# ZenGo-X/zk-paillier

Measured on AMD Instinct MI355X. Metric: RangeProofNi proofs/sec + verifies/sec, n=2048, batch=4096 per GPU (value = verifies/sec; proofs/sec in prove.value), higher is better.
Workload: dtype u32 (29-bit limbs, u64 accumulate)

## Files before the change

### zk-paillier_amd/csrc/kernels_basen.hpp

```cpp
#pragma once
#include "kernels_modexp.hpp"

#define ZKP_UNROLL_STR(x) #x
#define ZKP_UNROLL_(n) _Pragma(ZKP_UNROLL_STR(unroll n))
#define ZKP_UNROLL(n) ZKP_UNROLL_(n)
#ifndef ZKP_BN_ROW_UNROLL
#if ZKP_W == 9
#define ZKP_BN_ROW_UNROLL 8
#else
#define ZKP_BN_ROW_UNROLL 1
#endif
#endif
#ifndef ZKP_BN_ASM
#define ZKP_BN_ASM (ZKP_W == 36)
#endif
namespace zkp {
template <int G> constexpr bool BN_ASM_G = ZKP_BN_ASM && W == 36 && (G == 2 || G == 4);

template <int G> struct BnConst {
  static constexpr int L = Geo<G>::L;
  static constexpr int OFF_MT = 0, OFF_C3 = L, OFF_RRA = 2 * L, OFF_RRB = 3 * L, OFF_N = 4 * L, OFF_R2N = 5 * L, OFF_ONE = 6 * L, OFF_R1A = 7 * L, OFF_R1B = 8 * L, OFF_NI = 9 * L, OFF_OK = 9 * L + 1;
  static constexpr int WORDS = 9 * L + 4;
  static constexpr int STRIDE = WORDS + 2 * L;
};
// ... 533 lines not shown
  store_limbs_global<G>(tab + L, Y, g.gl);
  bn_stage<G>(g, g.A(), X);
  bn_stage<G>(g, g.B(), Y);
  const int msb = 31 - __clz(CAP);
#pragma unroll 1
  for (int b = msb - 1; b >= 0; b--) {
    bn_square<G>(g, X);
    if ((CAP >> b) & 1) {
      uint32_t A2[W], B2[W];
      bn_product<G>(g, A2, B2, tab, tab + L);
      bn_stage<G>(g, g.A(), A2);
      bn_stage<G>(g, g.B(), B2);
#pragma unroll
      for (int k = 0; k < W; k++) X[k] = A2[k];
    }
  }
  lds_load_block(Y, g.B() + g.gl * BLK);
  store_limbs_global<G>(out + BC::OFF_RRA, X, g.gl);
  store_limbs_global<G>(out + BC::OFF_RRB, Y, g.gl);
  store_limbs_global<G>(out + BC::OFF_R1A, OA, g.gl);
  store_limbs_global<G>(out + BC::OFF_R1B, OB, g.gl);
  if (g.gl == 0) {
    out[BC::OFF_OK] = ok ? 1u : 0u;
    if (!ok) atomicAnd(all_ok, 0u);
  }
  if (tag && up_tag && gid == 0 && g.gl == 0) {
    tag[1] = up_tag[5];
    __threadfence();
    tag[0] = (ok && up_tag[0] == SETUP_TAG_MAGIC) ? SETUP_TAG_MAGIC : 0u;
  }
}

template <int GS>
__global__ void __launch_bounds__(256, ZKP_WPE) k_expected(EncArgs a, uint32_t* __restrict__ expected, const uint32_t* __restrict__ bn_ok) {
  using CL = ConstLayout<GS>;
  using LL = LdsLayout<GS>;
  if (!*bn_ok) return;
  extern __shared__ __align__(16) uint32_t lds_raw[];
  Grp<GS> g;
  grp_init<GS>(g, lds_raw);
  const int kw = a.n_bits / 32;
  const uint64_t count = a.count_ptr ? (uint64_t)*a.count_ptr : a.count;
  const uint64_t stride = (uint64_t)gridDim.x * LL::GROUPS_PER_BLOCK;
  const uint64_t rounds = (count + stride - 1) / stride;
  const uint32_t* cst = a.consts;
  load_modulus_consts<GS>(g, cst);
  for (uint64_t rd = 0; rd < rounds; rd++) {
    const uint64_t idx = rd * stride + (uint64_t)blockIdx.x * LL::GROUPS_PER_BLOCK + (threadIdx.x / GS);
    const bool live = idx < count;
    const uint64_t item = live ? idx : count - 1;
    uint64_t b;
    bool mask_row;
    const uint32_t* pexp;
    if (a.mode == 2) { b = item; mask_row = a.cipher_x != nullptr; pexp = a.c1 + item * 2 * kw; }
    else {
      b = a.item_proof[item];
      const uint32_t rw = a.item_row[item];
      const uint64_t row = b * a.ef + (rw >> 1);
      mask_row = a.resp_kind[row] != 0;
      const bool use_c1 = mask_row ? (a.resp_j[row] == 1) : !(rw & 1);
      pexp = (use_c1 ? a.c1 : a.c2) + row * 2 * kw;
    }
    if (a.const_stride) {
      const uint64_t i0 = (a.mode == 0 && a.half && item >= a.half) ? item - a.half : item;
      cst = a.consts + (a.mode == 1 ? b : i0 / a.items_per_key) * a.const_stride;
      load_modulus_consts<GS>(g, cst);
    }
    const bool valid = cst[CL::OFF_ST] == 0;
    uint32_t A[W], R[W], Y[W];
    load_value<GS>(g, A, pexp, valid ? 2 * kw : 0);
    stage_const<GS>(g, cst + CL::OFF_R2);
    mm<GS>(g, R, A);
    {
      uint32_t t[W];
      load_value<GS>(g, t, a.cipher_x + b * 2 * kw, (mask_row && valid) ? 2 * kw : 0);
      if (!mask_row && valid && g.gl == 0) t[0] = 1;
      stageB<GS>(g, t);
    }
    mm<GS>(g, Y, R);
    stage_const<GS>(g, cst + CL::OFF_R2);
    mm<GS>(g, R, Y);
    stage_one<GS>(g);
    mm<GS>(g, Y, R);
    canonical_words<GS>(g, Y, cst + CL::OFF_N);
    if (live && mask_row) for (int w = g.gl; w < 2 * kw; w += GS) expected[item * 2 * kw + w] = g.words()[w];
  }
}

struct BnItem {
  const uint32_t* pm; const uint32_t* pr; const uint32_t* pexp; uint32_t* pout;
  uint64_t b; int mw, rw; bool mask_row;
};
__device__ __forceinline__ BnItem bn_item(const EncArgs& a, uint64_t item, const uint32_t* expected) {
  BnItem it{};
  const int kw = a.n_bits / 32;
  it.mw = kw; it.rw = kw;
  if (a.mode == 0) {
    const bool second = a.half && item >= a.half;
    const uint64_t i = second ? item - a.half : item;
    it.mw = a.m_words < 0 ? 0 : (a.m_words ? a.m_words : kw);
    it.rw = a.r_words ? a.r_words : kw;
    it.pm = (second ? a.m2 : a.m) + i * it.mw;
    it.pr = (second ? a.r2 : a.r) + i * it.rw;
    it.pout = (second ? a.out2 : a.out) + i * 2 * kw;
  } else if (a.mode == 2) {
    it.b = item;
    it.pm = a.m + item * kw;
    it.pr = a.r + item * kw;
    it.mask_row = a.cipher_x != nullptr;
    it.pexp = it.mask_row ? expected + item * 2 * kw : a.c1 + item * 2 * kw;
  } else {
    it.b = a.item_proof[item];
    const uint32_t rw = a.item_row[item];
    const uint64_t row = it.b * a.ef + (rw >> 1);
    it.mask_row = a.resp_kind[row] != 0;
    const bool second = (rw & 1) != 0;
    it.pm = (second ? a.resp_w2 : a.resp_w1) + row * kw;
    it.pr = (second ? a.resp_r2 : a.resp_r1) + row * kw;
// ... 568 lines not shown
```

### zk-paillier_amd/csrc/kernels_proofs.hpp

```cpp
#pragma once
#include "kernels_modexp.hpp"
#include "kernels_gcd.hpp"
#include "sha256_dev.hpp"

namespace zkp {

__device__ __forceinline__ int cmp_words(const uint32_t* a, const uint32_t* b, int n) {
  for (int i = n - 1; i >= 0; i--) {
    const uint32_t x = a[i], y = b[i];
    if (x != y) return x > y ? 1 : -1;
  }
  return 0;
}

__device__ __forceinline__ int challenge_bit(const uint8_t* e, uint32_t i) { return (e[i >> 3] >> (7 - (i & 7))) & 1; }

struct RangeHashArgs {
  const uint32_t* n; uint64_t n_stride;
  const uint32_t* c1; const uint32_t* c2; const uint32_t* range;
  uint32_t kw, ef; uint64_t batch;
  uint8_t* e;
  uint8_t* e_len;
  uint32_t* third;
  uint32_t* two_thirds;
// ... 243 lines not shown
  const uint8_t* db = reinterpret_cast<const uint8_t*>(s.row);
  int lead = 0;
  while (lead < 31 && db[lead] == 0) lead++;
  uint8_t* e = a.e + b * 32;
  for (int i = 0; i < 32; i++) e[i] = (i + lead < 32) ? db[i + lead] : 0;
  const int elen = 32 - lead;
  a.e_len[b] = (uint8_t)elen;
  a.verdict[b] = ((uint32_t)elen * 8 >= a.ef) ? a.ok_value : (uint8_t)ZKP_VERDICT_MALFORMED;
  if (!a.range) return;
  const uint32_t* rg = a.range + b * a.kw;
  uint32_t* t1 = a.third + b * a.kw;
  uint32_t* t2 = a.two_thirds + b * a.kw;
  uint64_t rem = 0;
  for (int w = (int)a.kw - 1; w >= 0; w--) {
    const uint64_t cur = (rem << 32) | rg[w];
    t1[w] = (uint32_t)(cur / 3);
    rem = cur % 3;
  }
  uint32_t carry = 0;
  for (uint32_t w = 0; w < a.kw; w++) { const uint32_t v = t1[w]; t2[w] = (v << 1) | carry; carry = v >> 31; }
}

#ifndef ZKP_TEMPLATE_KERNELS_ONLY
__global__ void __launch_bounds__(64) k_range_hash_wave(RangeHashArgs a) { range_hash_wave_body(a, (int)threadIdx.x, blockIdx.x); }
#endif

struct VerifyPlanArgs {
  const uint8_t* e; const uint8_t* resp_kind;
  const uint32_t* resp_w1; const uint32_t* resp_w2;
  const uint32_t* third; const uint32_t* two_thirds;
  uint32_t kw, ef; uint64_t batch;
  uint8_t* verdict;
  uint32_t* item_proof; uint32_t* item_row; unsigned long long* counter;
};

#ifndef ZKP_TEMPLATE_KERNELS_ONLY
__global__ void __launch_bounds__(256) k_verify_plan(VerifyPlanArgs a) {
  const uint64_t t = (uint64_t)blockIdx.x * 256 + threadIdx.x;
  const bool in = t < a.batch * a.ef;
  uint32_t nitems = 0;
  uint64_t b = 0; uint32_t i = 0;
  if (in && !a.e) {
    b = t / a.ef; i = (uint32_t)(t % a.ef);
    const int kind = a.resp_kind[t];
    nitems = kind == ZKP_RESP_OPEN ? 2 : kind == ZKP_RESP_MASK ? 1 : 0;
  } else if (in) {
    b = t / a.ef; i = (uint32_t)(t % a.ef);
    if (a.verdict[b] != ZKP_VERDICT_MALFORMED) {
      const int ei = challenge_bit(a.e + b * 32, i);
      const int kind = a.resp_kind[t];
      const uint32_t* T1 = a.third + b * a.kw;
      const uint32_t* T2 = a.two_thirds + b * a.kw;
      const uint32_t* w1 = a.resp_w1 + t * a.kw;
      if (!ei && kind == ZKP_RESP_OPEN) {
        const uint32_t* w2 = a.resp_w2 + t * a.kw;
        const int w1_T1 = cmp_words(w1, T1, a.kw), w2_T1 = cmp_words(w2, T1, a.kw);
        const bool flag = (w2_T1 < 0 && w1_T1 > 0 && cmp_words(w1, T2, a.kw) < 0) ||
                          (w1_T1 < 0 && w2_T1 > 0 && cmp_words(w2, T2, a.kw) < 0);
        if (!flag) a.verdict[b] = ZKP_VERDICT_REJECT;
        nitems = 2;
      } else if (ei && kind == ZKP_RESP_MASK) {
        if (cmp_words(w1, T1, a.kw) < 0 || cmp_words(w1, T2, a.kw) > 0) a.verdict[b] = ZKP_VERDICT_REJECT;
        nitems = 1;
      } else {
        a.verdict[b] = ZKP_VERDICT_REJECT;
      }
    }
  }
  if (!a.item_proof) return;
  const unsigned long long m2 = __ballot(nitems == 2), m1 = __ballot(nitems == 1);
  const int lane = threadIdx.x & 63;
  const unsigned long long lt = (1ull << lane) - 1;
  const uint32_t before = 2 * __popcll(m2 & lt) + __popcll(m1 & lt);
  const uint32_t total = 2 * __popcll(m2) + __popcll(m1);
  unsigned long long base = 0;
  if (lane == 0 && total) base = atomicAdd(a.counter, (unsigned long long)total);
  base = __shfl(base, 0);
  for (uint32_t k = 0; k < nitems; k++) {
    a.item_proof[base + before + k] = (uint32_t)b;
    a.item_row[base + before + k] = (i << 1) | k;
  }
}
#endif

struct VerdictMergeArgs {
  uint8_t* verdict; const uint8_t* enc_verdict; const uint8_t* e; const uint8_t* resp_kind; uint32_t ef; uint64_t batch;
};
#ifndef ZKP_TEMPLATE_KERNELS_ONLY
__global__ void __launch_bounds__(256) k_verdict_merge(VerdictMergeArgs a) {
  const uint64_t b = (uint64_t)blockIdx.x * 256 + threadIdx.x;
  if (b >= a.batch) return;
  const uint8_t v = a.verdict[b], ev = a.enc_verdict[b];
  if (v == ZKP_VERDICT_MALFORMED || ev == ZKP_VERDICT_ACCEPT) return;
  if (ev == ZKP_VERDICT_REJECT) { a.verdict[b] = ZKP_VERDICT_REJECT; return; }
  bool any = false;
  for (uint32_t i = 0; i < a.ef; i++) {
    const int ei = challenge_bit(a.e + b * 32, i), kind = a.resp_kind[b * a.ef + i];
    any = any || (!ei && kind == ZKP_RESP_OPEN) || (ei && kind == ZKP_RESP_MASK);
  }
  if (any) a.verdict[b] = ZKP_VERDICT_MALFORMED;
}
#endif

struct ResponseArgs {
  const uint32_t* consts; uint64_t const_stride;
  const uint32_t* x; const uint32_t* r;
  const uint32_t* w1; const uint32_t* w2; const uint32_t* r1; const uint32_t* r2;
  const uint8_t* e; const uint32_t* third; const uint32_t* two_thirds;
  uint8_t* resp_kind; uint8_t* resp_j; uint32_t* resp_w1; uint32_t* resp_r1; uint32_t* resp_w2; uint32_t* resp_r2;
  uint8_t* status;
  uint32_t kw, ef; uint64_t batch;
};

template <int G>
// ... 456 lines not shown
```

### zk-paillier_amd/csrc/zkp_api.hip

```cpp
#include <hip/hip_runtime.h>
#include <dlfcn.h>

#include <algorithm>
#include <cstdio>
#include <cstdlib>
#include <new>
#include <cstring>
#include <exception>
#include <mutex>
#include <string>
#include <thread>
#include <type_traits>
#include <vector>

#include "../../include/zkp_hip.h"
#include "../../include/zkp_hip_diag.h"
#include "kernels_modexp.hpp"
#include "kernels_proofs.hpp"
#include "kernels_inv.hpp"
#include "kernels_serde.hpp"
#include "kernels_serde_write.hpp"
#include "kernels_serde_scan.hpp"
#include "kernels_sample.hpp"
#include "kernels_coprime.hpp"
#include "route_plan.hpp"
#if ZKP_W == 36 || ZKP_W == 18 || ZKP_W == 9
#define ZKP_HAS_BASEN 1
#include "kernels_basen.hpp"
#include "kernels_basen_r2l.hpp"
#else
#define ZKP_HAS_BASEN 0
#endif

using namespace zkp;

struct DevBuf {
  void* p = nullptr;
  size_t cap = 0;
  uint32_t* tag = nullptr;
  uint64_t gen = 0, tag_gen = 0;
};

struct StageBlock { void* p; size_t cap; };

enum ScratchSlot : int {
  S_E = 0,
  S_ELEN = 1,
  S_T1 = 2, S_T2 = 3,
  S_IPROOF = 4, S_IROW = 5, S_COUNTER = 6,
  S_STATUS = 7,
  S_MGF = 8, S_PRIMES = 9,
  S_DLOG_E = 10,
  S_TMP1 = 11, S_TMP2 = 12, S_TMP3 = 13,
  S_SCHED = 15,
  S_TMP4 = 16, S_TMP5 = 17,
  S_WORK_COUNTER = 18,
  S_ENCV = 19,
  S_MP_NN = 20, S_MP_INVST = 21,
  S_MP_T0 = 22,
  S_MP_END = 32,
  S_CM_SUM = 34, S_CM_FLAGS = 35,
  S_CM_T0 = 36,
  S_CM_END = 44,
  S_SAMPLE_THIRD = 44, S_SAMPLE_META = 45, S_SAMPLE_STATUS = 46,
  S_RESIDUE = 47,
  S_COUNT = 48
};
static_assert(S_MP_T0 + 9 < S_MP_END && S_MP_END <= S_CM_SUM && S_CM_T0 + 7 < S_CM_END && S_CM_END <= S_SAMPLE_THIRD && S_RESIDUE < S_COUNT,
              "scratch slot runs overlap");

struct zkp_ctx {
  std::vector<StageBlock> stage_free;
  std::vector<std::pair<void*, size_t>> last_wiped;
  uint32_t* setup_flag = nullptr;
  uint32_t* setup_flag_host = nullptr;
  int device = 0;
  hipStream_t stream = nullptr;
  bool owns_stream = true;
  RouteKnobs route;
  const struct LatEngine* eng[2] = {nullptr, nullptr};
  zkp_ctx* eng_ctx[2] = {nullptr, nullptr};
  const struct LatEngine* lat = nullptr;
  zkp_ctx* lat_ctx = nullptr;
  int last_geometry = 0;
  hipStream_t side = nullptr;
  hipEvent_t ev_fork = nullptr, ev_join = nullptr;
  bool side_busy = false;
  hipStream_t copy = nullptr;
  std::vector<hipEvent_t> ev_pipe;
  bool copy_busy = false;
  int last_host_blocks = 0;
  uint64_t scan_fast = 0, scan_fallback = 0;
  hipEvent_t ev_scan[5] = {nullptr, nullptr, nullptr, nullptr, nullptr};
  int scan_phases = 0;
  zkp_ctx* split_ctx = nullptr;
  hipStream_t split_stream = nullptr;
  hipEvent_t ev_split[2] = {nullptr, nullptr};
  int last_split = 0;
  int key_cache = 1;
  int host_chunks = -1;
  std::string err;
  DevBuf consts, consts2, table, scratch[S_COUNT];
  DevBuf bn_ncst, bn_consts, bn_table, bn_expected, bn_raw, bn_left;
  int bn_occ[2][2] = {{0, 0}, {0, 0}};
  int bn_last_g = 0;
  bool bn_last_per_key = false;
  bool bn_last_r2l = false;
  int bn_last_r2l_lanes = 0;
  const RangeHashArgs* fuse_hash = nullptr;
  bool fuse_hash_taken = false;
  DevBuf bn_flag;
  bool timing = false;
  std::vector<std::pair<hipEvent_t, hipEvent_t>> ev;
  size_t ev_used = 0;
  uint64_t timed_launches = 0, timed_modexps = 0;
  static constexpr size_t PINNED_SLOTS = 4096;
  unsigned long long* pinned_counts = nullptr;
  size_t pinned_used = 0;
};

#define HIPCHK(ctx, call)                                                                         \
  do {                                                                                            \
    hipError_t e_ = (call);                                                                       \
    if (e_ != hipSuccess) {                                                                       \
      (ctx)->err = std::string(#call) + ": " + hipGetErrorString(e_);                             \
      return e_ == hipErrorOutOfMemory ? ZKP_ENOMEM : ZKP_EDEVICE;                                \
    }                                                                                             \
  } while (0)

static int32_t zkp_caught(zkp_ctx* c, int32_t st, const char* what) noexcept {
  if (c) { try { c->err = what; } catch (...) {} }
  return st;
}
#define ZKP_CATCH(ctx)                                                                                         \
  catch (const std::bad_alloc&) { return zkp_caught((ctx), ZKP_ENOMEM, "out of host memory"); }               \
  catch (const std::exception& e_) { return zkp_caught((ctx), ZKP_EDEVICE, e_.what()); }                      \
  catch (...) { return zkp_caught((ctx), ZKP_EDEVICE, "unknown exception"); }

#define ZKP_LAT_FUNCS(X)                                                                                                        \
  X(zkp_ctx_create_on_stream) X(zkp_ctx_destroy) X(zkp_last_error_string) X(zkp_build_limbs_per_lane) X(zkp_ctx_release_staging) \
  X(zkp_timing_reset) X(zkp_timing_get) X(zkp_modexp_batch) X(zkp_paillier_enc_batch) X(zkp_paillier_enc_check_batch)            \
  X(zkp_range_ni_prove_batch) X(zkp_range_ni_verify_batch) X(zkp_range_generate_encrypted_pairs_batch) X(zkp_range_challenge_batch)                           \
  X(zkp_range_verifier_output_batch) X(zkp_correct_key_ni_verify_batch) X(zkp_dlog_prove_batch) X(zkp_dlog_verify_batch)         \
// ... 347 lines not shown
  *out = (unsigned long long*)b.p;
  return ZKP_OK;
}

static int32_t side_stream(zkp_ctx* c) {
  if (c->side) return ZKP_OK;
  HIPCHK(c, hipEventCreateWithFlags(&c->ev_fork, hipEventDisableTiming));
  HIPCHK(c, hipEventCreateWithFlags(&c->ev_join, hipEventDisableTiming));
  HIPCHK(c, hipStreamCreateWithFlags(&c->side, hipStreamNonBlocking));
  return ZKP_OK;
}

template <int G, class K> static int32_t table_for(zkp_ctx* c, K kernel, uint64_t items, unsigned* blocks_out) {
  using LL = LdsLayout<G>;
  const uint64_t need = (items + LL::GROUPS_PER_BLOCK - 1) / LL::GROUPS_PER_BLOCK;
  const unsigned blocks = (unsigned)std::max<uint64_t>(1, std::min<uint64_t>(need, (uint64_t)resident_blocks<G>(c, kernel)));
  *blocks_out = blocks;
  return ensure(c, c->table, (size_t)blocks * LL::GROUPS_PER_BLOCK * TAB * Geo<G>::L * sizeof(uint32_t));
}

constexpr bool PAIR_LADDER_BUILD = ZKP_W <= 9;

#if ZKP_HAS_BASEN
constexpr int BN_GA = 72 / W, BN_GB = 144 / W;
#ifdef ZKP_SPLIT_TU
extern template __global__ void zkp::k_enc_basen<BN_GA>(EncArgs, const uint32_t*, uint32_t*, uint32_t*);
extern template __global__ void zkp::k_enc_basen<BN_GB>(EncArgs, const uint32_t*, uint32_t*, uint32_t*);
extern template __global__ void zkp::k_enc_basen_keys<BN_GA>(EncArgs, const uint32_t*, const uint32_t*, uint32_t*, uint32_t*);
extern template __global__ void zkp::k_enc_basen_keys<BN_GB>(EncArgs, const uint32_t*, const uint32_t*, uint32_t*, uint32_t*);
extern template __global__ void zkp::k_basen_finish<BN_GA>(EncArgs, const uint32_t*, const uint32_t*, int, const uint32_t*, const uint32_t*, const uint32_t*);
extern template __global__ void zkp::k_basen_finish<BN_GB>(EncArgs, const uint32_t*, const uint32_t*, int, const uint32_t*, const uint32_t*, const uint32_t*);
extern template __global__ void zkp::k_setup_basen<BN_GA>(const uint32_t*, uint32_t*, uint64_t, uint32_t*, const uint32_t*, uint32_t*);
extern template __global__ void zkp::k_setup_basen<BN_GB>(const uint32_t*, uint32_t*, uint64_t, uint32_t*, const uint32_t*, uint32_t*);
extern template __global__ void zkp::k_expected<2 * BN_GA>(EncArgs, uint32_t*, const uint32_t*);
extern template __global__ void zkp::k_expected<2 * BN_GB>(EncArgs, uint32_t*, const uint32_t*);
extern template __global__ void zkp::k_diag_basen<BN_GA>(const uint32_t*, int, const uint32_t*, const uint32_t*, const uint32_t*, const uint32_t*, uint32_t*, uint32_t*);
extern template __global__ void zkp::k_diag_basen<BN_GB>(const uint32_t*, int, const uint32_t*, const uint32_t*, const uint32_t*, const uint32_t*, uint32_t*, uint32_t*);
#endif
constexpr size_t BASEN_DIAG_LDS = 4096;
static int enc_form_from_env() {
  const char* e = std::getenv("ZKP_BASEN");
  if (e && e[0] == '0') return ZKP_ENC_FORM_N2;
  if (e && e[0] == 's') return ZKP_ENC_FORM_SHARED;
  if (e && e[0] == 'a') return ZKP_ENC_FORM_ALWAYS;
  return ZKP_ENC_FORM_AUTO;
}
template <int G> static int32_t basen_prepare(zkp_ctx* c, const uint32_t* n, uint64_t n_stride, uint64_t nkeys, uint32_t n_bits) {
  int32_t st = run_setup<G>(c, n, n_stride, (int)(n_bits / 32), 0, nkeys, c->bn_ncst);
  if (st) return st;
  if ((st = ensure(c, c->bn_consts, (size_t)(nkeys + 1) * BnConst<G>::STRIDE * sizeof(uint32_t)))) return st;
  HIPCHK(c, hipMemsetAsync((char*)c->bn_consts.p + (size_t)nkeys * BnConst<G>::STRIDE * sizeof(uint32_t), 0, BnConst<G>::STRIDE * sizeof(uint32_t), c->stream));
  if ((st = ensure(c, c->bn_flag, 64))) return st;
  HIPCHK(c, hipMemsetD32Async((hipDeviceptr_t)c->bn_flag.p, 1, 2, c->stream));
  constexpr unsigned GPB = 64 / G;
  uint32_t* tag = nullptr;
  if ((st = setup_tag(c, c->bn_consts, nkeys, &tag))) return st;
  hipLaunchKernelGGL(k_setup_basen<G>, dim3((unsigned)((nkeys + GPB - 1) / GPB)), dim3(64), GPB * BN_SETUP_LDS_WORDS * sizeof(uint32_t), c->stream,
                     (const uint32_t*)c->bn_ncst.p, (uint32_t*)c->bn_consts.p, nkeys, (uint32_t*)c->bn_flag.p, tag ? (const uint32_t*)c->bn_ncst.tag : nullptr, tag);
  HIPCHK(c, hipGetLastError());
  return ZKP_OK;
}
template <int G> static int basen_occupancy(zkp_ctx* c, bool per_key) {
  int& per_cu = c->bn_occ[per_key ? 1 : 0][G == BN_GB ? 1 : 0];
  if (!per_cu) {
    const hipError_t e = per_key ? hipOccupancyMaxActiveBlocksPerMultiprocessor(&per_cu, k_enc_basen_keys<G>, 256, BnLds<G>::BYTES_PER_BLOCK)
                                 : hipOccupancyMaxActiveBlocksPerMultiprocessor(&per_cu, k_enc_basen<G>, 256, BnLds<G>::BYTES_PER_BLOCK);
    if (e != hipSuccess || per_cu < 1) per_cu = 1;
  }
  return per_cu;
}
template <int GS> static bool launch_basen(zkp_ctx* c, const EncArgs& a_in, EncArgs* rest) {
  if constexpr (GS != 2 * BN_GA && GS != 2 * BN_GB) { (void)c; (void)a_in; (void)rest; return false; }
  else {
    constexpr int G = GS / 2;
    using BL = BnLds<G>;
    static_assert(HASH_WAVE_BLOCKS == HW_BLOCKS, "route_plan.hpp names the wave hash's full footprint");
    EncArgs a = a_in;
    const int kw = a.n_bits / 32;
    const bool per_key = a.n_stride != 0;
    c->bn_last_g = 0;
    BasenShape shape;
    shape.lanes = G; shape.per_key = per_key; shape.key_stride_fits = a.n_stride == (uint64_t)kw; shape.n_bits = a.n_bits; shape.mode = a.mode;
    shape.count = a.count; shape.listed = a.count_ptr != nullptr; shape.has_sched = a.sched != nullptr; shape.operands_fit = a.m_words <= kw && a.r_words <= kw;
    shape.hashes_offered = c->fuse_hash != nullptr; shape.hashes = c->fuse_hash ? c->fuse_hash->batch : 0;
    shape.groups_per_block = BL::GROUPS_PER_BLOCK; shape.per_cu = basen_occupancy<G>(c, per_key);
    const BasenPlan plan = basen_plan(c->route, shape);
    if (!plan.take) return false;
    uint64_t nkeys = 1;
    if (per_key) {
      const uint64_t items = (a.mode == 0 && a.half) ? a.half : a.count;
      nkeys = a.mode == 1 ? a.count / (2 * (uint64_t)a.ef) : (items + a.items_per_key - 1) / a.items_per_key;
      if (nkeys == 0) return false;
    }
    auto give_up = [&]() { c->err.clear(); *rest = a_in; return false; };
    if (basen_prepare<G>(c, a.n, a.n_stride, nkeys, (uint32_t)a.n_bits)) return give_up();
    const uint64_t need = (a.count + BL::GROUPS_PER_BLOCK - 1) / BL::GROUPS_PER_BLOCK;
    const size_t entries = per_key ? BN_KEYS_TAB_ENTRIES : BN_TAB_ENTRIES;
    if (!plan.r2l && ensure(c, c->bn_table, (size_t)plan.blocks * BL::GROUPS_PER_BLOCK * entries * 2 * Geo<G>::L * sizeof(uint32_t))) return give_up();
    if (ensure(c, c->bn_raw, (size_t)a.count * 2 * Geo<G>::L * sizeof(uint32_t))) return give_up();
    const uint32_t* ok = per_key ? (const uint32_t*)c->bn_flag.p + 1 : (const uint32_t*)c->bn_consts.p + BnConst<G>::OFF_OK;
    if (per_key) {
      if (ensure(c, c->bn_left, 16 + (size_t)a.count * sizeof(uint32_t))) return give_up();
      if (hipMemsetAsync(c->bn_left.p, 0, 16, c->stream) != hipSuccess) return give_up();
      a.left_count = (unsigned long long*)c->bn_left.p;
      a.left_list = (uint32_t*)((char*)c->bn_left.p + 16);
      rest->remap = a.left_list; rest->remap_count = a.left_count;
      rest->work_counter = a.work_counter + 1;
    }
    const bool products = a.mode == 1 || (a.mode == 2 && a.cipher_x);
    if (products) {
      if (ensure(c, c->bn_expected, (size_t)a.count * 2 * kw * sizeof(uint32_t))) return give_up();
      using LS = LdsLayout<GS>;
      const uint64_t eneed = (a.count + LS::GROUPS_PER_BLOCK - 1) / LS::GROUPS_PER_BLOCK;
      const unsigned eblocks = (unsigned)std::max<uint64_t>(1, std::min<uint64_t>(eneed, 2ull * c->route.cus));
      hipLaunchKernelGGL(k_expected<GS>, dim3(eblocks), dim3(256), LS::BYTES_PER_BLOCK, c->stream, a, (uint32_t*)c->bn_expected.p, ok);
    }
    c->bn_last_g = G; c->bn_last_per_key = per_key; c->bn_last_r2l = plan.r2l;
#if ZKP_W == 9
    if (plan.r2l) {
      if constexpr (G == 8) {
        c->bn_last_r2l_lanes = plan.r2l_lanes;
        RangeHashArgs h{};
        size_t dyn = 0;
        if (plan.hash_blocks) {
          h = *c->fuse_hash;
          c->fuse_hash_taken = true;
          if (plan.r2l_lanes != 36) h.wave_blocks = (uint32_t)plan.hash_blocks;
          dyn = (size_t)(plan.hash_blocks == 16 ? hw_lds_words<16>((int)h.kw) : hw_lds_words<HW_BLOCKS>((int)h.kw)) * sizeof(uint32_t);
        }
        const dim3 grid((unsigned)(h.batch + plan.enc_wgs));
        if (plan.r2l_lanes == 36) hipLaunchKernelGGL(k_enc_basen_r2l5, grid, dim3(320), dyn, c->stream, a, (const uint32_t*)c->bn_consts.p, (uint32_t*)c->bn_raw.p, h);
        else if (plan.r2l_lanes == 8) hipLaunchKernelGGL(k_enc_basen_r2l<9>, grid, dim3(64), dyn, c->stream, a, (const uint32_t*)c->bn_consts.p, (uint32_t*)c->bn_raw.p, h);
        else hipLaunchKernelGGL(k_enc_basen_r2l<6>, grid, dim3(64), dyn, c->stream, a, (const uint32_t*)c->bn_consts.p, (uint32_t*)c->bn_raw.p, h);
      }
    } else
#endif
    if (per_key)
      hipLaunchKernelGGL(k_enc_basen_keys<G>, dim3(plan.blocks), dim3(256), BL::BYTES_PER_BLOCK, c->stream, a, (const uint32_t*)c->bn_consts.p, (const uint32_t*)c->bn_consts.p + (size_t)nkeys * BnConst<G>::STRIDE, (uint32_t*)c->bn_table.p,
                         (uint32_t*)c->bn_raw.p);
    else
      hipLaunchKernelGGL(k_enc_basen<G>, dim3(plan.blocks), dim3(256), BL::BYTES_PER_BLOCK, c->stream, a, (const uint32_t*)c->bn_consts.p, (uint32_t*)c->bn_table.p,
                         (uint32_t*)c->bn_raw.p);
    const unsigned fblocks = (unsigned)std::max<uint64_t>(1, std::min<uint64_t>(need, 8ull * c->route.cus));
    hipLaunchKernelGGL(k_basen_finish<G>, dim3(fblocks), dim3(256), BL::BYTES_PER_BLOCK, c->stream, a, (const uint32_t*)c->bn_consts.p, ok, per_key ? 1 : 0,
                       (const uint32_t*)c->bn_raw.p, (const uint32_t*)c->bn_expected.p, (const uint32_t*)c->bn_consts.p + (size_t)nkeys * BnConst<G>::STRIDE);
    return true;
  }
}
#endif
// ... 592 lines not shown
```

### zk-paillier_amd/csrc/zkp_api_proofs.inc

```

enum : unsigned { RA_RANGE = 1, RA_CIPHERTEXT = 2, RA_PAIRS = 4, RA_RESP = 8 };
static bool range_args_ok(const zkp_range_ni_proofs* p, unsigned need = RA_RANGE | RA_CIPHERTEXT | RA_PAIRS | RA_RESP) {
  if (!p) return false;
  if (!key_bits_ok(p->n_bits)) return false;
  if (p->batch > (1ull << 24) || p->error_factor > 256) return false;
  if (p->n_stride != 0 && p->n_stride != p->n_bits / 32) return false;
  if (p->batch == 0) return true;
  if (!p->n || ((need & RA_RANGE) && !p->range) || ((need & RA_CIPHERTEXT) && !p->ciphertext)) return false;
  if (p->error_factor && (need & RA_PAIRS) && (!p->c1 || !p->c2)) return false;
  if (p->error_factor && (need & RA_RESP) && (!p->resp_kind || !p->resp_j || !p->resp_w1 || !p->resp_r1 || !p->resp_w2 || !p->resp_r2)) return false;
  return true;
}

static zkp_range_ni_proofs range_slice(const zkp_range_ni_proofs& p, size_t EF, uint64_t lo, uint64_t count) {
  const size_t kw = p.n_bits / 32;
  zkp_range_ni_proofs q = p;
  q.batch = count;
  if (q.n) q.n += lo * p.n_stride;
  if (q.range) q.range += lo * kw;
  if (q.ciphertext) q.ciphertext += lo * 2 * kw;
  for (uint32_t** a : {&q.c1, &q.c2}) if (*a) *a += lo * EF * 2 * kw;
  for (uint8_t** a : {&q.resp_kind, &q.resp_j}) if (*a) *a += lo * EF;
  for (uint32_t** a : {&q.resp_w1, &q.resp_r1, &q.resp_w2, &q.resp_r2}) if (*a) *a += lo * EF * kw;
  return q;
// ... 368 lines not shown
  ZKP_ROUTE_ENC(c, p ? p->batch * 2 * p->error_factor : 0, p ? 2 * p->n_bits : 0, p && p->n_stride == 0, zkp_range_generate_encrypted_pairs_batch, p, w, flags)
  return range_prove_entry(c, "zkp_range_generate_encrypted_pairs_batch", p, w, p ? p->error_factor : 0, 1, nullptr, nullptr, nullptr, nullptr, nullptr, flags);
} ZKP_CATCH(c)
extern "C" int32_t zkp_range_generate_proof_batch(zkp_ctx* c, const zkp_range_ni_proofs* p, const zkp_range_ni_witness* w, const uint8_t* e,
                                                  const uint8_t* e_len, uint8_t* out_status, uint32_t flags) try {
  if (c && (!e || !e_len)) { c->err = "zkp_range_generate_proof_batch: the challenge is an input"; return ZKP_EINVAL; }
  return range_prove_entry(c, "zkp_range_generate_proof_batch", p, w, p ? p->error_factor : 0, 2, e, e_len, nullptr, nullptr, out_status, flags);
} ZKP_CATCH(c)

extern "C" int32_t zkp_range_challenge_batch(zkp_ctx* c, const zkp_range_ni_proofs* p, uint8_t* out_e, uint8_t* out_e_len, uint32_t flags) try {
  ZKP_ROUTE(c, p ? p->batch * 2 * p->error_factor : 0, p ? 2 * p->n_bits : 0, zkp_range_challenge_batch, p, out_e, out_e_len, flags)
  if (!c) return ZKP_EINVAL;
  if (!range_args_ok(p, RA_PAIRS) || (p->batch && (!out_e || !out_e_len))) { c->err = "zkp_range_challenge_batch: invalid argument"; return ZKP_EINVAL; }
  if (p->batch == 0) return ZKP_OK;
  HIPCHK(c, hipSetDevice(c->device));
  const size_t kw = p->n_bits / 32, B = p->batch, rows = B * p->error_factor;
  Stage s(c, flags);
  zkp_range_ni_proofs d = *p;
  d.n = s.in(p->n, p->n_stride ? B * kw : kw);
  d.c1 = (uint32_t*)s.in((const uint32_t*)p->c1, rows * 2 * kw); d.c2 = (uint32_t*)s.in((const uint32_t*)p->c2, rows * 2 * kw);
  d.range = nullptr;
  uint8_t* de = s.out(out_e, B * 32);
  uint8_t* dl = s.out(out_e_len, B);
  int32_t st = s.st;
  if (!st) st = ensure(c, c->scratch[S_STATUS], B);
  if (!st) st = range_hash<GA>(c, d, de, dl, (uint8_t*)c->scratch[S_STATUS].p, 0);
  const int32_t fin = s.finish();
  return st ? st : fin;
} ZKP_CATCH(c)

struct FuseHashScope {
  zkp_ctx* c;
  int unwinding;
  FuseHashScope(zkp_ctx* c_, const RangeHashArgs* h) : c(c_), unwinding(std::uncaught_exceptions()) { c->fuse_hash = h; c->fuse_hash_taken = false; }
  ~FuseHashScope() {
    c->fuse_hash = nullptr;
    if (std::uncaught_exceptions() > unwinding) c->fuse_hash_taken = false;
  }
  FuseHashScope(const FuseHashScope&) = delete;
  FuseHashScope& operator=(const FuseHashScope&) = delete;
};

template <int G>
static int32_t range_verify_impl(zkp_ctx* c, const zkp_range_ni_proofs& p, uint8_t* verdict, const uint8_t* e_in = nullptr,
                                 const uint8_t* e_len_in = nullptr) {
  using CL = ConstLayout<G>;
  const uint32_t kw = p.n_bits / 32, EF = p.error_factor;
  const uint64_t nkeys = p.n_stride ? p.batch : 1, rows = p.batch * EF;
  int32_t st;
  if ((st = run_setup<G>(c, p.n, p.n_stride, (int)kw, 1, nkeys, c->consts))) return st;
  if ((st = ensure(c, c->scratch[S_E], p.batch * 32))) return st;
  if ((st = ensure(c, c->scratch[S_ELEN], p.batch))) return st;
  const uint64_t enc_blocks = (2 * rows + LdsLayout<G>::GROUPS_PER_BLOCK - 1) / LdsLayout<G>::GROUPS_PER_BLOCK;
  const char* two_env = std::getenv("ZKP_TWO_STREAMS");
  const bool two = rows != 0 && !e_in && two_streams(c->route, enc_blocks, two_env ? (two_env[0] == '1' ? 1 : 0) : -1);
  const bool fuse = two && c->route.fuse_hash_on && p.batch < (uint64_t)c->route.cus && basen_r2l_takes_hashes<G>(c, p.n_stride, p.n_bits, 2 * rows, p.batch);
  hipStream_t hs = c->stream;
  uint8_t* enc_verdict = verdict;
  if (two) {
    if ((st = ensure(c, c->scratch[S_ENCV], p.batch))) return st;
    enc_verdict = (uint8_t*)c->scratch[S_ENCV].p;
    HIPCHK(c, hipMemsetAsync(enc_verdict, ZKP_VERDICT_ACCEPT, p.batch, c->stream));
  }
  if (two && !fuse) {
    if ((st = side_stream(c))) return st;
    HIPCHK(c, hipEventRecord(c->ev_fork, c->stream));
    HIPCHK(c, hipStreamWaitEvent(c->side, c->ev_fork, 0));
    c->side_busy = true;
    hs = c->side;
  }
  RangeHashArgs fused_hash{};
  if ((st = range_hash<G>(c, p, (uint8_t*)c->scratch[S_E].p, (uint8_t*)c->scratch[S_ELEN].p, verdict, ZKP_VERDICT_ACCEPT, e_in, e_len_in, hs, fuse ? &fused_hash : nullptr))) return st;
  if (rows == 0) return ZKP_OK;
  if ((st = ensure(c, c->scratch[S_IPROOF], 2 * rows * 4))) return st;
  if ((st = ensure(c, c->scratch[S_IROW], 2 * rows * 4))) return st;
  if ((st = ensure(c, c->scratch[S_COUNTER], 16))) return st;
  HIPCHK(c, hipMemsetAsync(c->scratch[S_COUNTER].p, 0, 16, c->stream));
  VerifyPlanArgs v{(const uint8_t*)c->scratch[S_E].p, p.resp_kind, p.resp_w1, p.resp_w2, (const uint32_t*)c->scratch[S_T1].p,
                   (const uint32_t*)c->scratch[S_T2].p, kw, EF, p.batch, verdict, (uint32_t*)c->scratch[S_IPROOF].p,
                   (uint32_t*)c->scratch[S_IROW].p, (unsigned long long*)c->scratch[S_COUNTER].p};
  const dim3 plan_grid((unsigned)((rows + 255) / 256));
  VerifyPlanArgs pred = v; pred.item_proof = nullptr; pred.item_row = nullptr; pred.counter = nullptr;
  if (two) {
    if (!fuse) {
      hipLaunchKernelGGL(k_verify_plan, plan_grid, dim3(256), 0, c->side, pred);
      HIPCHK(c, hipGetLastError());
      HIPCHK(c, hipEventRecord(c->ev_join, c->side));
    }
    VerifyPlanArgs list = v; list.e = nullptr; list.verdict = nullptr;
    hipLaunchKernelGGL(k_verify_plan, plan_grid, dim3(256), 0, c->stream, list);
  } else {
    hipLaunchKernelGGL(k_verify_plan, plan_grid, dim3(256), 0, c->stream, v);
  }
  HIPCHK(c, hipGetLastError());
  unsigned blocks = 0;
  if ((st = table_for<G>(c, k_enc<G, true>, 2 * rows, &blocks))) return st;
  EncArgs a{};
  a.n = p.n; a.n_stride = p.n_stride; a.consts = (const uint32_t*)c->consts.p; a.const_stride = p.n_stride ? (uint64_t)CL::WORDS : 0;
  a.table = (uint32_t*)c->table.p; a.count = 2 * rows ; a.n_bits = (int)p.n_bits; a.mode = 1;
  a.item_proof = (const uint32_t*)c->scratch[S_IPROOF].p; a.item_row = (const uint32_t*)c->scratch[S_IROW].p;
  a.resp_w1 = p.resp_w1; a.resp_r1 = p.resp_r1; a.resp_w2 = p.resp_w2; a.resp_r2 = p.resp_r2; a.resp_kind = p.resp_kind; a.resp_j = p.resp_j;
  a.c1 = p.c1; a.c2 = p.c2; a.cipher_x = p.ciphertext; a.verdict = enc_verdict;
  a.count_ptr = (const unsigned long long*)c->scratch[S_COUNTER].p; a.ef = EF;
  if (p.n_stride == 0 && !pair_ladder(c->route, G, a.count) && (st = build_schedule(c, p.n, p.n_bits, &a.sched))) return st;
  if ((st = fresh_work_counter(c, &a.work_counter))) return st;
  {
    TimedRegion tr(c, 0);
    FuseHashScope fh(c, fuse ? &fused_hash : nullptr);
    launch_k_enc<G>(c, blocks, a);
  }
  HIPCHK(c, hipGetLastError());
  if (fuse) {
    if (!c->fuse_hash_taken) {
      hipLaunchKernelGGL(k_range_hash_wave, dim3((unsigned)p.batch), dim3(64), hw_lds_words((int)kw) * sizeof(uint32_t), c->stream, fused_hash);
      HIPCHK(c, hipGetLastError());
    }
    hipLaunchKernelGGL(k_verify_plan, plan_grid, dim3(256), 0, c->stream, pred);
    HIPCHK(c, hipGetLastError());
  }
  if (two) {
    if (!fuse) {
      HIPCHK(c, hipStreamWaitEvent(c->stream, c->ev_join, 0));
      c->side_busy = false;
    }
    VerdictMergeArgs m{verdict, enc_verdict, (const uint8_t*)c->scratch[S_E].p, p.resp_kind, EF, p.batch};
    hipLaunchKernelGGL(k_verdict_merge, dim3((unsigned)((p.batch + 255) / 256)), dim3(256), 0, c->stream, m);
    HIPCHK(c, hipGetLastError());
  }
  if (c->timing && c->pinned_counts && c->pinned_used < zkp_ctx::PINNED_SLOTS)
    HIPCHK(c, hipMemcpyAsync(&c->pinned_counts[c->pinned_used++], c->scratch[S_COUNTER].p, 8, hipMemcpyDeviceToHost, c->stream));
  return ZKP_OK;
}

static int32_t range_verify_entry(zkp_ctx* c, const zkp_range_ni_proofs* p, const uint8_t* e_in, const uint8_t* e_len_in, uint8_t* out_verdict, uint32_t flags);
extern "C" int32_t zkp_range_ni_verify_batch(zkp_ctx* c, const zkp_range_ni_proofs* p, uint8_t* out_verdict, uint32_t flags) try {
  ZKP_RANGE_SPLIT_RESET(c)
#ifndef ZKP_SECONDARY_ENGINE
  if (const RangeSplit sp = (p && out_verdict && range_args_ok(p)) ? range_split_plan(c, p, 2 * (uint64_t)p->error_factor, true) : RangeSplit(); sp.head && range_split_ready(c)) {
    const uint64_t head = sp.head, tail = p->batch - head;
    auto part = [&](const LatEngine* e, zkp_ctx* ec, uint64_t lo, uint64_t count) {
      const zkp_range_ni_proofs q = range_slice(*p, p->error_factor, lo, count);
// ... 450 lines not shown
```

### zk-paillier_amd/csrc/zkp_kernels_basen.hip

```cpp
#define ZKP_TEMPLATE_KERNELS_ONLY
#include "../../include/zkp_hip.h"
#include "kernels_basen.hpp"

namespace zkp {
constexpr int BN_GA = 72 / W, BN_GB = 144 / W;
template __global__ void k_enc_basen<BN_GA>(EncArgs, const uint32_t*, uint32_t*, uint32_t*);
template __global__ void k_enc_basen<BN_GB>(EncArgs, const uint32_t*, uint32_t*, uint32_t*);
template __global__ void k_enc_basen_keys<BN_GA>(EncArgs, const uint32_t*, const uint32_t*, uint32_t*, uint32_t*);
template __global__ void k_enc_basen_keys<BN_GB>(EncArgs, const uint32_t*, const uint32_t*, uint32_t*, uint32_t*);
template __global__ void k_basen_finish<BN_GA>(EncArgs, const uint32_t*, const uint32_t*, int, const uint32_t*, const uint32_t*, const uint32_t*);
template __global__ void k_basen_finish<BN_GB>(EncArgs, const uint32_t*, const uint32_t*, int, const uint32_t*, const uint32_t*, const uint32_t*);
template __global__ void k_setup_basen<BN_GA>(const uint32_t*, uint32_t*, uint64_t, uint32_t*, const uint32_t*, uint32_t*);
template __global__ void k_setup_basen<BN_GB>(const uint32_t*, uint32_t*, uint64_t, uint32_t*, const uint32_t*, uint32_t*);
template __global__ void k_expected<2 * BN_GA>(EncArgs, uint32_t*, const uint32_t*);
template __global__ void k_expected<2 * BN_GB>(EncArgs, uint32_t*, const uint32_t*);
template __global__ void k_diag_basen<BN_GA>(const uint32_t*, int, const uint32_t*, const uint32_t*, const uint32_t*, const uint32_t*, uint32_t*, uint32_t*);
template __global__ void k_diag_basen<BN_GB>(const uint32_t*, int, const uint32_t*, const uint32_t*, const uint32_t*, const uint32_t*, uint32_t*, uint32_t*);
}
```

Before: 3542.

## Compact mask-row list for expected products and restructure k_expected loop

The verify planner now also writes a compacted list of mask-row items with its own counter, so k_expected iterates only over rows that need an expected value instead of all 2*rows items. The kernel is recast as a single-mm step loop that reuses one operand buffer and caches R^3, which keeps code size and register use small. The grid for k_expected is sized from measured occupancy rather than a fixed 2 per CU. The main encryption launch can wait on the side-stream join event, which moves where the two streams synchronise. The cost is an extra atomic and scatter in the planner, plus more complex control flow.

```diff
diff --git a/zk-paillier_amd/csrc/kernels_basen.hpp b/zk-paillier_amd/csrc/kernels_basen.hpp
--- a/zk-paillier_amd/csrc/kernels_basen.hpp
+++ b/zk-paillier_amd/csrc/kernels_basen.hpp
@@ -589,58 +589,74 @@
 }
 
 template <int GS>
-__global__ void __launch_bounds__(256, ZKP_WPE) k_expected(EncArgs a, uint32_t* __restrict__ expected, const uint32_t* __restrict__ bn_ok) {
+__global__ void __launch_bounds__(256, ZKP_WPE) k_expected(EncArgs a, uint32_t* __restrict__ expected, const uint32_t* __restrict__ bn_ok,
+                                                           const uint32_t* __restrict__ mask_items, const unsigned long long* __restrict__ mask_count) {
   using CL = ConstLayout<GS>;
   using LL = LdsLayout<GS>;
   if (!*bn_ok) return;
+  const uint64_t count = a.mode == 1 ? (uint64_t)*mask_count : a.count;
+  if (count == 0) return;
   extern __shared__ __align__(16) uint32_t lds_raw[];
   Grp<GS> g;
   grp_init<GS>(g, lds_raw);
   const int kw = a.n_bits / 32;
-  const uint64_t count = a.count_ptr ? (uint64_t)*a.count_ptr : a.count;
   const uint64_t stride = (uint64_t)gridDim.x * LL::GROUPS_PER_BLOCK;
   const uint64_t rounds = (count + stride - 1) / stride;
+  const bool per_key = a.const_stride != 0;
   const uint32_t* cst = a.consts;
   load_modulus_consts<GS>(g, cst);
-  for (uint64_t rd = 0; rd < rounds; rd++) {
-    const uint64_t idx = rd * stride + (uint64_t)blockIdx.x * LL::GROUPS_PER_BLOCK + (threadIdx.x / GS);
-    const bool live = idx < count;
-    const uint64_t item = live ? idx : count - 1;
-    uint64_t b;
-    bool mask_row;
-    const uint32_t* pexp;
-    if (a.mode == 2) { b = item; mask_row = a.cipher_x != nullptr; pexp = a.c1 + item * 2 * kw; }
-    else {
-      b = a.item_proof[item];
-      const uint32_t rw = a.item_row[item];
-      const uint64_t row = b * a.ef + (rw >> 1);
-      mask_row = a.resp_kind[row] != 0;
-      const bool use_c1 = mask_row ? (a.resp_j[row] == 1) : !(rw & 1);
-      pexp = (use_c1 ? a.c1 : a.c2) + row * 2 * kw;
-    }
-    if (a.const_stride) {
-      const uint64_t i0 = (a.mode == 0 && a.half && item >= a.half) ? item - a.half : item;
-      cst = a.consts + (a.mode == 1 ? b : i0 / a.items_per_key) * a.const_stride;
-      load_modulus_consts<GS>(g, cst);
+  enum { ST_R3 = 0, ST_EX = 1, ST_UP = 2, ST_DOWN = 3 };
+  const int item_first = per_key ? ST_R3 : ST_EX;
+  uint32_t X[W], R3[W];
+  uint64_t rd = 0, item = 0, b = 0;
+  bool live = false;
+  int step = ST_R3;
+#pragma unroll 1
+  for (;;) {
+    if (step == item_first) {
+      const uint64_t idx = rd * stride + (uint64_t)blockIdx.x * LL::GROUPS_PER_BLOCK + (threadIdx.x / GS);
+      live = idx < count;
+      const uint64_t at = live ? idx : count - 1;
+      item = a.mode == 1 ? (uint64_t)mask_items[at] : at;
+      b = a.mode == 1 ? (uint64_t)a.item_proof[item] : item;
+      if (per_key) {
+        cst = a.consts + (a.mode == 1 ? b : item / a.items_per_key) * a.const_stride;
+        load_modulus_consts<GS>(g, cst);
+      }
     }
     const bool valid = cst[CL::OFF_ST] == 0;
-    uint32_t A[W], R[W], Y[W];
-    load_value<GS>(g, A, pexp, valid ? 2 * kw : 0);
-    stage_const<GS>(g, cst + CL::OFF_R2);
-    mm<GS>(g, R, A);
-    {
+    if (step == ST_R3) {
+      load_limbs_global<GS>(X, cst + CL::OFF_R2, g.gl);
+      if (!valid) {
+#pragma unroll
+        for (int k = 0; k < W; k++) X[k] = 0;
+      }
+      stage_const<GS>(g, cst + CL::OFF_R2);
+    } else if (step == ST_EX) {
+      const uint32_t* pexp;
+      if (a.mode == 1) {
+        const uint64_t row = b * a.ef + (a.item_row[item] >> 1);
+        pexp = (a.resp_j[row] == 1 ? a.c1 : a.c2) + row * 2 * kw;
+      } else pexp = a.c1 + item * 2 * kw;
       uint32_t t[W];
-      load_value<GS>(g, t, a.cipher_x + b * 2 * kw, (mask_row && valid) ? 2 * kw : 0);
-      if (!mask_row && valid && g.gl == 0) t[0] = 1;
+      load_value<GS>(g, t, a.cipher_x + b * 2 * kw, valid ? 2 * kw : 0);
       stageB<GS>(g, t);
-    }
-    mm<GS>(g, Y, R);
-    stage_const<GS>(g, cst + CL::OFF_R2);
-    mm<GS>(g, R, Y);
-    stage_one<GS>(g);
-    mm<GS>(g, Y, R);
-    canonical_words<GS>(g, Y, cst + CL::OFF_N);
-    if (live && mask_row) for (int w = g.gl; w < 2 * kw; w += GS) expected[item * 2 * kw + w] = g.words()[w];
+      load_value<GS>(g, X, pexp, valid ? 2 * kw : 0);
+    } else if (step == ST_UP) {
+      stageB<GS>(g, R3);
+    } else {
+      stage_one<GS>(g);
+    }
+    mm<GS>(g, X, X);
+    if (step == ST_R3) {
+#pragma unroll
+      for (int k = 0; k < W; k++) R3[k] = X[k];
+    }
+    if (step != ST_DOWN) { step++; continue; }
+    canonical_words<GS>(g, X, cst + CL::OFF_N);
+    if (live) for (int w = g.gl; w < 2 * kw; w += GS) expected[item * 2 * kw + w] = g.words()[w];
+    if (++rd == rounds) break;
+    step = item_first;
   }
 }
 
diff --git a/zk-paillier_amd/csrc/kernels_proofs.hpp b/zk-paillier_amd/csrc/kernels_proofs.hpp
--- a/zk-paillier_amd/csrc/kernels_proofs.hpp
+++ b/zk-paillier_amd/csrc/kernels_proofs.hpp
@@ -299,6 +299,7 @@
   uint32_t kw, ef; uint64_t batch;
   uint8_t* verdict;
   uint32_t* item_proof; uint32_t* item_row; unsigned long long* counter;
+  uint32_t* mask_items; unsigned long long* mask_count;
 };
 
 #ifndef ZKP_TEMPLATE_KERNELS_ONLY
@@ -340,13 +341,19 @@
   const unsigned long long lt = (1ull << lane) - 1;
   const uint32_t before = 2 * __popcll(m2 & lt) + __popcll(m1 & lt);
   const uint32_t total = 2 * __popcll(m2) + __popcll(m1);
-  unsigned long long base = 0;
-  if (lane == 0 && total) base = atomicAdd(a.counter, (unsigned long long)total);
+  const uint32_t mtotal = a.mask_items ? __popcll(m1) : 0;
+  unsigned long long base = 0, mbase = 0;
+  if (lane == 0) {
+    if (total) base = atomicAdd(a.counter, (unsigned long long)total);
+    if (mtotal) mbase = atomicAdd(a.mask_count, (unsigned long long)mtotal);
+  }
   base = __shfl(base, 0);
+  mbase = __shfl(mbase, 0);
   for (uint32_t k = 0; k < nitems; k++) {
     a.item_proof[base + before + k] = (uint32_t)b;
     a.item_row[base + before + k] = (i << 1) | k;
   }
+  if (mtotal && nitems == 1) a.mask_items[mbase + __popcll(m1 & lt)] = (uint32_t)(base + before);
 }
 #endif
 
diff --git a/zk-paillier_amd/csrc/zkp_api.hip b/zk-paillier_amd/csrc/zkp_api.hip
--- a/zk-paillier_amd/csrc/zkp_api.hip
+++ b/zk-paillier_amd/csrc/zkp_api.hip
@@ -52,6 +52,7 @@
   S_MGF = 8, S_PRIMES = 9,
   S_DLOG_E = 10,
   S_TMP1 = 11, S_TMP2 = 12, S_TMP3 = 13,
+  S_MASK_ITEMS = 14,
   S_SCHED = 15,
   S_TMP4 = 16, S_TMP5 = 17,
   S_WORK_COUNTER = 18,
@@ -59,6 +60,7 @@
   S_MP_NN = 20, S_MP_INVST = 21,
   S_MP_T0 = 22,
   S_MP_END = 32,
+  S_MASK_COUNT = 33,
   S_CM_SUM = 34, S_CM_FLAGS = 35,
   S_CM_T0 = 36,
   S_CM_END = 44,
@@ -103,12 +105,14 @@
   DevBuf consts, consts2, table, scratch[S_COUNT];
   DevBuf bn_ncst, bn_consts, bn_table, bn_expected, bn_raw, bn_left;
   int bn_occ[2][2] = {{0, 0}, {0, 0}};
+  int ex_occ[2] = {0, 0};
   int bn_last_g = 0;
   bool bn_last_per_key = false;
   bool bn_last_r2l = false;
   int bn_last_r2l_lanes = 0;
   const RangeHashArgs* fuse_hash = nullptr;
   bool fuse_hash_taken = false;
+  hipEvent_t enc_after = nullptr;
   DevBuf bn_flag;
   bool timing = false;
   std::vector<std::pair<hipEvent_t, hipEvent_t>> ev;
@@ -522,8 +526,8 @@
 extern template __global__ void zkp::k_basen_finish<BN_GB>(EncArgs, const uint32_t*, const uint32_t*, int, const uint32_t*, const uint32_t*, const uint32_t*);
 extern template __global__ void zkp::k_setup_basen<BN_GA>(const uint32_t*, uint32_t*, uint64_t, uint32_t*, const uint32_t*, uint32_t*);
 extern template __global__ void zkp::k_setup_basen<BN_GB>(const uint32_t*, uint32_t*, uint64_t, uint32_t*, const uint32_t*, uint32_t*);
-extern template __global__ void zkp::k_expected<2 * BN_GA>(EncArgs, uint32_t*, const uint32_t*);
-extern template __global__ void zkp::k_expected<2 * BN_GB>(EncArgs, uint32_t*, const uint32_t*);
+extern template __global__ void zkp::k_expected<2 * BN_GA>(EncArgs, uint32_t*, const uint32_t*, const uint32_t*, const unsigned long long*);
+extern template __global__ void zkp::k_expected<2 * BN_GB>(EncArgs, uint32_t*, const uint32_t*, const uint32_t*, const unsigned long long*);
 extern template __global__ void zkp::k_diag_basen<BN_GA>(const uint32_t*, int, const uint32_t*, const uint32_t*, const uint32_t*, const uint32_t*, uint32_t*, uint32_t*);
 extern template __global__ void zkp::k_diag_basen<BN_GB>(const uint32_t*, int, const uint32_t*, const uint32_t*, const uint32_t*, const uint32_t*, uint32_t*, uint32_t*);
 #endif
@@ -558,6 +562,17 @@
     if (e != hipSuccess || per_cu < 1) per_cu = 1;
   }
   return per_cu;
+}
+#ifndef ZKP_EXPECTED_GRID
+#define ZKP_EXPECTED_GRID 0
+#endif
+template <int GS> static uint64_t expected_resident(zkp_ctx* c) {
+  if (ZKP_EXPECTED_GRID == 2) return ~0ull;
+  int& per_cu = c->ex_occ[GS == 2 * BN_GB ? 1 : 0];
+  if (!per_cu) {
+    if (hipOccupancyMaxActiveBlocksPerMultiprocessor(&per_cu, k_expected<GS>, 256, LdsLayout<GS>::BYTES_PER_BLOCK) != hipSuccess || per_cu < 1) per_cu = 1;
+  }
+  return (uint64_t)(ZKP_EXPECTED_GRID == 1 ? 1 : per_cu) * c->route.cus;
 }
 template <int GS> static bool launch_basen(zkp_ctx* c, const EncArgs& a_in, EncArgs* rest) {
   if constexpr (GS != 2 * BN_GA && GS != 2 * BN_GB) { (void)c; (void)a_in; (void)rest; return false; }
@@ -601,10 +616,15 @@
     if (products) {
       if (ensure(c, c->bn_expected, (size_t)a.count * 2 * kw * sizeof(uint32_t))) return give_up();
       using LS = LdsLayout<GS>;
-      const uint64_t eneed = (a.count + LS::GROUPS_PER_BLOCK - 1) / LS::GROUPS_PER_BLOCK;
-      const unsigned eblocks = (unsigned)std::max<uint64_t>(1, std::min<uint64_t>(eneed, 2ull * c->route.cus));
-      hipLaunchKernelGGL(k_expected<GS>, dim3(eblocks), dim3(256), LS::BYTES_PER_BLOCK, c->stream, a, (uint32_t*)c->bn_expected.p, ok);
+      const bool listed = a.mode == 1;
+      const uint64_t eitems = listed ? a.count / 2 : a.count;
+      const uint64_t eneed = (eitems + LS::GROUPS_PER_BLOCK - 1) / LS::GROUPS_PER_BLOCK;
+      const unsigned eblocks = (unsigned)std::max<uint64_t>(1, std::min<uint64_t>(eneed, expected_resident<GS>(c)));
+      hipLaunchKernelGGL(k_expected<GS>, dim3(eblocks), dim3(256), LS::BYTES_PER_BLOCK, c->stream, a, (uint32_t*)c->bn_expected.p, ok,
+                         listed ? (const uint32_t*)c->scratch[S_MASK_ITEMS].p : nullptr, listed ? (const unsigned long long*)c->scratch[S_MASK_COUNT].p : nullptr);
     }
+    if (c->enc_after && !plan.r2l && (uint64_t)plan.blocks >= (uint64_t)shape.per_cu * c->route.cus &&
+        hipStreamWaitEvent(c->stream, c->enc_after, 0) != hipSuccess) return give_up();
     c->bn_last_g = G; c->bn_last_per_key = per_key; c->bn_last_r2l = plan.r2l;
 #if ZKP_W == 9
     if (plan.r2l) {
diff --git a/zk-paillier_amd/csrc/zkp_api_proofs.inc b/zk-paillier_amd/csrc/zkp_api_proofs.inc
--- a/zk-paillier_amd/csrc/zkp_api_proofs.inc
+++ b/zk-paillier_amd/csrc/zkp_api_proofs.inc
@@ -424,9 +424,12 @@
 struct FuseHashScope {
   zkp_ctx* c;
   int unwinding;
-  FuseHashScope(zkp_ctx* c_, const RangeHashArgs* h) : c(c_), unwinding(std::uncaught_exceptions()) { c->fuse_hash = h; c->fuse_hash_taken = false; }
+  FuseHashScope(zkp_ctx* c_, const RangeHashArgs* h, hipEvent_t side_done = nullptr) : c(c_), unwinding(std::uncaught_exceptions()) {
+    c->fuse_hash = h; c->fuse_hash_taken = false; c->enc_after = side_done;
+  }
   ~FuseHashScope() {
     c->fuse_hash = nullptr;
+    c->enc_after = nullptr;
     if (std::uncaught_exceptions() > unwinding) c->fuse_hash_taken = false;
   }
   FuseHashScope(const FuseHashScope&) = delete;
@@ -468,9 +471,13 @@
   if ((st = ensure(c, c->scratch[S_IROW], 2 * rows * 4))) return st;
   if ((st = ensure(c, c->scratch[S_COUNTER], 16))) return st;
   HIPCHK(c, hipMemsetAsync(c->scratch[S_COUNTER].p, 0, 16, c->stream));
+  if ((st = ensure(c, c->scratch[S_MASK_ITEMS], rows * 4))) return st;
+  if ((st = ensure(c, c->scratch[S_MASK_COUNT], 16))) return st;
+  HIPCHK(c, hipMemsetAsync(c->scratch[S_MASK_COUNT].p, 0, 16, c->stream));
   VerifyPlanArgs v{(const uint8_t*)c->scratch[S_E].p, p.resp_kind, p.resp_w1, p.resp_w2, (const uint32_t*)c->scratch[S_T1].p,
                    (const uint32_t*)c->scratch[S_T2].p, kw, EF, p.batch, verdict, (uint32_t*)c->scratch[S_IPROOF].p,
-                   (uint32_t*)c->scratch[S_IROW].p, (unsigned long long*)c->scratch[S_COUNTER].p};
+                   (uint32_t*)c->scratch[S_IROW].p, (unsigned long long*)c->scratch[S_COUNTER].p,
+                   (uint32_t*)c->scratch[S_MASK_ITEMS].p, (unsigned long long*)c->scratch[S_MASK_COUNT].p};
   const dim3 plan_grid((unsigned)((rows + 255) / 256));
   VerifyPlanArgs pred = v; pred.item_proof = nullptr; pred.item_row = nullptr; pred.counter = nullptr;
   if (two) {
@@ -498,7 +505,7 @@
   if ((st = fresh_work_counter(c, &a.work_counter))) return st;
   {
     TimedRegion tr(c, 0);
-    FuseHashScope fh(c, fuse ? &fused_hash : nullptr);
+    FuseHashScope fh(c, fuse ? &fused_hash : nullptr, two && !fuse ? c->ev_join : nullptr);
     launch_k_enc<G>(c, blocks, a);
   }
   HIPCHK(c, hipGetLastError());
diff --git a/zk-paillier_amd/csrc/zkp_kernels_basen.hip b/zk-paillier_amd/csrc/zkp_kernels_basen.hip
--- a/zk-paillier_amd/csrc/zkp_kernels_basen.hip
+++ b/zk-paillier_amd/csrc/zkp_kernels_basen.hip
@@ -12,8 +12,8 @@
 template __global__ void k_basen_finish<BN_GB>(EncArgs, const uint32_t*, const uint32_t*, int, const uint32_t*, const uint32_t*, const uint32_t*);
 template __global__ void k_setup_basen<BN_GA>(const uint32_t*, uint32_t*, uint64_t, uint32_t*, const uint32_t*, uint32_t*);
 template __global__ void k_setup_basen<BN_GB>(const uint32_t*, uint32_t*, uint64_t, uint32_t*, const uint32_t*, uint32_t*);
-template __global__ void k_expected<2 * BN_GA>(EncArgs, uint32_t*, const uint32_t*);
-template __global__ void k_expected<2 * BN_GB>(EncArgs, uint32_t*, const uint32_t*);
+template __global__ void k_expected<2 * BN_GA>(EncArgs, uint32_t*, const uint32_t*, const uint32_t*, const unsigned long long*);
+template __global__ void k_expected<2 * BN_GB>(EncArgs, uint32_t*, const uint32_t*, const uint32_t*, const unsigned long long*);
 template __global__ void k_diag_basen<BN_GA>(const uint32_t*, int, const uint32_t*, const uint32_t*, const uint32_t*, const uint32_t*, uint32_t*, uint32_t*);
 template __global__ void k_diag_basen<BN_GB>(const uint32_t*, int, const uint32_t*, const uint32_t*, const uint32_t*, const uint32_t*, uint32_t*, uint32_t*);
 }
```

Result: no change. 3539 (-0.1%).
